# lym01803/FinalProject-LosslessImageCompression

Hardware: AMD Instinct MI355X
Metric: encode+decode Mpixels/s (imagenet64, bit-exact round trip) (higher is better)
Workload: dtype f32

## Files before the change

### finalproject-losslessimagecompression_amd/csrc/conv3_dx3.hip

```cpp
#include <hip/hip_runtime.h>
#include <stdint.h>
#include <stdlib.h>
#include <string.h>

#include <type_traits>
#include <utility>

#include "idf_cdf.h"
#include "idf_codec_internal.h"
#include "wino_common.h"

#pragma clang fp contract(off)

namespace idf {

typedef float d4 __attribute__((ext_vector_type(4)));
typedef _Float16 e4 __attribute__((ext_vector_type(4)));
typedef _Float16 e8 __attribute__((ext_vector_type(8)));
typedef unsigned int v4u __attribute__((ext_vector_type(4)));
typedef __bf16 b8 __attribute__((ext_vector_type(8)));

struct Dx3Args {
  const uint16_t* xs;
  int64_t P;
// ... 1062 lines not shown
                                                       const float* __restrict__ x, int64_t ld_x,
                                                       uint16_t* __restrict__ xb,
                                                       uint32_t* __restrict__ zero, int32_t nzero) {
  const int nq = ((c1 + 15) / 16 * 16 - c0) / 4;
  const int64_t g = (int64_t)blockIdx.x * blockDim.x + threadIdx.x;
  if (g < nzero) zero[g] = 0u;
  if (g >= P * nq) return;
  const int64_t pix = g / nq;
  const int c = c0 + 4 * (int)(g - pix * nq);
  d4 v = d4{0.f, 0.f, 0.f, 0.f};
  if (c < c1) v = *(const d4*)(x + pix * ld_x + c);
  typedef __bf16 b4 __attribute__((ext_vector_type(4)));
  *(b4*)((char*)xb + ((int64_t)(c >> 4) * P + pix) * 32 + (c & 15) * 2) = __builtin_convertvector(v, b4);
}

struct Dx3Plan {
  int ok, pitch, plane_kib, nbx, nby, ch, seg, segw, nseg, gut, wp, hp, nf, ngroup, split, tilew,
      xskip;
};

static int dx3_gcd(int a, int b) { return b ? dx3_gcd(b, a % b) : a; }

static Dx3Plan dx3_plan(int H, int W, int N, bool bf = false) {
  Dx3Plan p = {};
  p.tilew = 16;
  if (H < 1 || W < 1 || N < 1 || N > 1024) return p;
  const int nft = (N + 15) / 16;
  p.nf = nft <= 4 ? nft : 4;
  p.ngroup = (nft + p.nf - 1) / p.nf;
  if (W % 16 == 0) {
// ... 165 lines not shown
}

extern "C" int idf_dx3_head_init(void* stream, int64_t P, int32_t C0, const float* x, int64_t ld_x,
                                 const float* w, int32_t ldw, const float* bias, int32_t n_head,
                                 float* acc) {
  if (P <= 0) return P < 0 ? IDF_ERR_ARG : IDF_OK;
  if (!x || !w || !bias || !acc || n_head < 1 || n_head > 16 || C0 < 0 || C0 > 64 || (C0 & 3) ||
      (ld_x & 3) || (uintptr_t)x % 16 || (uintptr_t)acc % 16 || ldw < C0 || (ldw & 3) ||
      (uintptr_t)w % 16)
    return IDF_ERR_ARG;
  hipLaunchKernelGGL(dx3_head_init_kernel, dim3((unsigned)((P + 255) / 256)), dim3(256), 0,
                     (hipStream_t)stream, P, C0, x, ld_x, w, ldw, bias, n_head, acc);
  return idf_last_error();
}
#endif

static bool dxb_plan_ok(const Dx3Plan& p) {
  return p.ok && p.nf <= 3 && p.ngroup == 1 && (p.pitch == 18 || p.pitch == 10);
}

extern "C" int idf_conv3x3_dxb_supported(int32_t H, int32_t W, int32_t N) {
  return dxb_plan_ok(dx3_plan(H, W, N, true)) ? 1 : 0;
}

static bool dx3_plan_generic() {
  const char* e = getenv("IDF_DX3_PLAN");
  return e && !strcmp(e, "generic");
}

static int dx3_args(Dx3Args& g, Dx3Launch& sh, bool ml, bool bf, int32_t B, int32_t H, int32_t W,
// ... 283 lines not shown
```

### finalproject-losslessimagecompression_amd/csrc/flow_kernels.hip

```cpp
#include <hip/hip_runtime.h>
#include <stdint.h>

#include <algorithm>
#include <vector>

#include "idf_cdf.h"
#include "idf_codec_internal.h"

#pragma clang fp contract(off)

namespace idf {

typedef float floatx4 __attribute__((ext_vector_type(4)));

enum { MODE_DENSE = 0, MODE_CONV3 = 1 };
enum { EPI_STORE = 0, EPI_ACT = 1, EPI_COUPLE_ADD = 2, EPI_COUPLE_SUB = 3, EPI_PRIOR = 4,
       EPI_ACT_FOLD = 5 };

struct GemmArgs {
  int64_t P;
  int32_t K;
  int32_t N;
  const float* A;
  int64_t lda;
// ... 554 lines not shown
    t->used++;
  }
}

enum { COPY_NONE = 0, COPY_BF16_SHADOW, COPY_DX3_SPLIT, COPY_DXB };

struct BlockPlan {
  int8_t kind[IDF_MAX_DEPTH];
  bool wx3_first[IDF_MAX_DEPTH];
  bool fused;
  int head, head_init;
  int copy;
  int n_dx3;
  int dx3_nft;
  int conv_launches, setup_launches, head_launches;
  int64_t ld16, sh16;
  int nslab_xs;
  int64_t xs_bytes, off, need, hoff, bytes;
};

static int dense_block_plan(const IdfDenseBlock* blk, int32_t B, int32_t H, int32_t W, bool head,
                            BlockPlan* pl) {
  *pl = {};
  const int64_t P = (int64_t)B * H * W;
  const int depth = blk->depth;
  const bool dxb = blk->bf16 && blk->fold && blk->dxb && depth > 0 &&
                   idf_conv3x3_dxb_supported(H, W, blk->g_pad);
  bool dx3 = blk->fold && blk->wx3 && blk->dx3 && !blk->bf16 &&
             idf_conv3x3_dx3_supported(H, W, blk->g_pad);
  int n_dx3 = 0;
  while (dx3 && n_dx3 < depth && blk->dx3_w[n_dx3]) ++n_dx3;
  for (int i = n_dx3; dx3 && i < depth; ++i)
    if (blk->dx3_w[i]) return IDF_ERR_ARG;
  dx3 = dx3 && n_dx3 > 0;
// ... 37 lines not shown
  const bool wino = blk->fold && blk->wino && idf_conv3x3_wino_supported(H, W);
  for (int i = 0; i < depth; ++i) {
    int k = IDF_KIND_FOLD_GEMM;
    if (!blk->fold) k = IDF_KIND_UNFOLD;
    else if (dxb) k = IDF_KIND_DXB;
    else if (blk->bf16) k = IDF_KIND_BF16;
    else if (dx3 && i < n_dx3) k = IDF_KIND_DX3;
    else if (wino && blk->wino_u[i]) k = blk->wx3 && blk->wx3_u[i] ? IDF_KIND_WX3 : IDF_KIND_WINO;
    else if (blk->halo) k = IDF_KIND_HALO;
    pl->kind[i] = (int8_t)k;
    pl->wx3_first[i] = k == IDF_KIND_WX3 && (i == 0 || (dx3 && i == n_dx3));
  }
  pl->conv_launches = pl->fused ? 1 : blk->fold ? depth : 2 * depth;
  pl->setup_launches = (pl->copy != COPY_NONE) + (pl->head_init == IDF_HEAD_INIT_OWN_LAUNCH);
  pl->head_launches = pl->head == IDF_PLAN_HEAD_GEMM;
  return IDF_OK;
}

static bool block_args_ok(const IdfDenseBlock* blk, int32_t B, int32_t H, int32_t W) {
  return blk && blk->depth >= 0 && blk->depth <= IDF_MAX_DEPTH && B >= 0 && H >= 1 && W >= 1;
}

extern "C" int64_t idf_dense_block_dx3_tmp_bytes(const IdfDenseBlock* blk, int32_t B, int32_t H,
                                                  int32_t W) {
  BlockPlan pl;
  return block_args_ok(blk, B, H, W) && !dense_block_plan(blk, B, H, W, true, &pl) ? pl.bytes : -1;
}

extern "C" int idf_dense_block_plan(const IdfDenseBlock* blk, int32_t B, int32_t H, int32_t W,
                                    int32_t with_head, int32_t out[IDF_BLOCK_PLAN_N]) {
// ... 2 lines not shown
  if (!block_args_ok(blk, B, H, W)) return IDF_ERR_ARG;
  BlockPlan pl;
  if (int rc = dense_block_plan(blk, B, H, W, with_head != 0, &pl)) return rc;
  out[IDF_BLOCK_PLAN_FUSED] = pl.fused;
  out[IDF_BLOCK_PLAN_HEAD] = pl.head;
  out[IDF_BLOCK_PLAN_HEAD_INIT] = pl.head_init;
  out[IDF_BLOCK_PLAN_N_DX3] = pl.n_dx3;
  out[IDF_BLOCK_PLAN_CONV_LAUNCHES] = pl.conv_launches;
  out[IDF_BLOCK_PLAN_SETUP_LAUNCHES] = pl.setup_launches;
  out[IDF_BLOCK_PLAN_HEAD_LAUNCHES] = pl.head_launches;
  for (int i = 0; i < blk->depth; ++i) {
    out[IDF_BLOCK_PLAN_KIND0 + i] = pl.kind[i];
    if (pl.wx3_first[i]) out[IDF_BLOCK_PLAN_WX3_FIRST] |= (int32_t)(1u << i);
  }
  return IDF_OK;
}

static int dense_block_run_fused(void* stream, const IdfDenseBlock* blk, const BlockPlan& pl,
                                 int32_t B, int32_t H, int32_t W, float* feat, int64_t ld_feat,
                                 uint16_t* xs, const IdfDx3Head* hd, IdfTimer* timer) {
  const bool dxb = pl.copy == COPY_DXB;
  const int64_t P = (int64_t)B * H * W;
  int32_t C[16];
  const uint16_t* w[16];
  float ys[16];
  const float *b3[16], *vt[16], *bfu[16];
  double fl = 0.0;
  for (int i = 0; i < blk->depth; ++i) {
    C[i] = blk->k_in[i];
    w[i] = dxb ? blk->dxb_w[i] : blk->dx3_w[i];
// ... 29 lines not shown
  BlockPlan pl;
  if (int rc = dense_block_plan(blk, B, H, W, head != nullptr, &pl)) return rc;
  const int64_t tmp_floats = P * ld_tmp;
  const bool direct = pl.copy == COPY_DX3_SPLIT || pl.copy == COPY_DXB;
  if (pl.sh16 > tmp_floats || pl.bytes > tmp_floats * 4 || (direct && (uintptr_t)tmp % 256))
    return IDF_ERR_WORKSPACE;
  uint16_t* const xs = (uint16_t*)tmp;
  float* const ws = tmp + pl.sh16;
  char* const dws = (char*)tmp + pl.off;
  float* const hacc = pl.head == IDF_PLAN_HEAD_FUSED ? (float*)((char*)tmp + pl.hoff) : nullptr;
  const int c0 = blk->k_in[0];
  uint32_t* const ctr = pl.need > 0 ? (uint32_t*)dws : nullptr;
  const int32_t nctr =
      pl.need > 0 ? (int32_t)(idf_conv3x3_dx3_counter_bytes(B, H, W, blk->g_pad) / 4) : 0;
  int rc = IDF_OK;
  switch (pl.copy) {
    case COPY_BF16_SHADOW:
      rc = idf_f32_to_bf16_cols(stream, P, c0, (c0 + 7) / 8 * 8, feat, ld_feat, xs, pl.ld16);
      break;
    case COPY_DXB:
      rc = idf_dxb_cols(stream, P, 0, c0, feat, ld_feat, xs, pl.nslab_xs, ctr, nctr);
      break;
    case COPY_DX3_SPLIT:
      rc = pl.head_init == IDF_HEAD_INIT_IN_SPLIT
               ? idf_dx3_split_cols_head(stream, P, c0, feat, ld_feat, xs, pl.nslab_xs,
                                         blk->range_flag, ctr, nctr, blk->wh, blk->ldwh, blk->bh,
                                         blk->n_head, hacc)
               : idf_dx3_split_cols(stream, P, 0, c0, feat, ld_feat, xs, pl.nslab_xs,
                                    blk->range_flag, ctr, nctr);
      break;
  }
// ... 263 lines not shown
```

### finalproject-losslessimagecompression_amd/csrc/idf_codec_internal.h

```cpp
#pragma once
#include <hip/hip_runtime.h>
#include <stdint.h>

#include "../../include/idf_codec.h"

struct IdfDx3BlockDesc {
  int32_t bf;
  int32_t B, H, W, nlayers, N, nft, ldv, act, nslab_xs;
  float slope;
  uint16_t* xs;
  const int32_t* C;
  const uint16_t* const* w;
  const float* yscale;
  const float* const* b3;
  const float* const* vtap;
  const float* const* bfull;
  float* feat;
  int64_t ld_feat;
  uint32_t* flag;
  const IdfDx3Head* head;
  const float* hx;
  int64_t hld_x;
  int32_t hc0;
  const float* hb;
};
int idf_dx3_block_launch(void* stream, const IdfDx3BlockDesc* d);

#define IDF_FREQ_SCALE_ZERO ((int32_t)0x80000000)

static inline int idf_last_error() {
  hipError_t e = hipGetLastError();
  return e == hipSuccess ? IDF_OK : IDF_ERR_HIP;
}

namespace idf {

__device__ __forceinline__ int xcd_contiguous(int bid, int nwg) {
#ifdef IDF_XCD_OFF
  return bid;
#endif
  const int q = nwg / 8, r = nwg % 8;
// ... 38 lines not shown
```

### finalproject-losslessimagecompression_amd/idfcodec/_lib.py

```python
from __future__ import annotations

import ctypes
import os

import torch

HERE = os.path.dirname(os.path.abspath(__file__))
PKG = os.path.dirname(HERE)
REPO = os.path.dirname(PKG)
LIB_PATH = os.environ.get("IDF_LIB_PATH") or os.path.join(HERE, "libidfcodec.so")
HEADER = os.path.join(REPO, "include", "idf_codec.h")

IDF_OK = 0
IDF_ERR_UNSUPPORTED = 4
ERR_NAMES = {1: "IDF_ERR_ARG", 2: "IDF_ERR_HIP", 3: "IDF_ERR_WORKSPACE", 4: "IDF_ERR_UNSUPPORTED"}

STREAM_SCALE_ZERO = 1
STREAM_FREQ_ZERO = 2
STREAM_NEG_CDF = 4
STREAM_UNDERFLOW = 8
STREAM_OUT_OF_WINDOW = 16
STREAM_WORDS_LEFT = 32

ACT = {"ReLU": 0, "LeakyReLU": 1, "Tanh": 2, "None": 3}
# ... 10 lines not shown

class IdfDenseBlock(ctypes.Structure):
    _fields_ = [
        ("depth", i32), ("act", i32), ("slope", f32), ("g_pad", i32), ("g_alloc", i32),
        ("k_in", i32 * (MAX_DEPTH + 1)), ("n1_alloc", i32 * MAX_DEPTH), ("ldw1", i32 * MAX_DEPTH),
        ("ldw3", i32 * MAX_DEPTH), ("w1", P * MAX_DEPTH), ("b1", P * MAX_DEPTH),
        ("w3", P * MAX_DEPTH), ("b3", P * MAX_DEPTH), ("n_head", i32), ("nh_alloc", i32),
        ("ldwh", i32), ("wh", P), ("bh", P),
        ("c_real", i32 * (MAX_DEPTH + 1)), ("g_real", i32 * MAX_DEPTH),
        ("fold", i32), ("ldv", i32), ("vtap", P * MAX_DEPTH), ("bfull", P * MAX_DEPTH),
        ("halo", i32), ("wino", i32), ("wino_nft", i32), ("wino_u", P * MAX_DEPTH),
        ("bf16", i32), ("wb16", P * MAX_DEPTH),
        ("wx3", i32), ("wx3_yscale", f32 * MAX_DEPTH), ("wx3_u", P * MAX_DEPTH), ("range_flag", P),
        ("dx3", i32), ("dx3_yscale", f32 * MAX_DEPTH), ("dx3_w", P * MAX_DEPTH),
        ("fuse_head", i32), ("keep_feat", i32),
        ("dxb", i32), ("dxb_w", P * MAX_DEPTH), ("fuse_layers", i32),
    ]


class IdfHeadOut(ctypes.Structure):
    _fields_ = [
        ("mode", i32), ("out", P), ("ld_out", i64), ("base", P), ("ld_base", i64),
        ("n_mean", i32), ("mean", P), ("logscale", P), ("scale", P),
    ]


class IdfDx3Head(ctypes.Structure):
    _fields_ = [
        ("w", P), ("ldw", i32), ("n_head", i32), ("acc", P), ("last", i32), ("skip_f32", i32),
        ("out", IdfHeadOut),
    ]
# ... 13 lines not shown
                                                    P]),
    "idf_gather_words": (ctypes.c_int, [P, i64, P, P, P, P, P]),
    "idf_rans_host_workspace_bytes": (i64, [i64, i64]),
    "idf_rans_encode_on": (ctypes.c_int, [P, P, i64, P, i64, P, P, P, P, P, P]),
    "idf_rans_decode_on": (ctypes.c_int, [P, P, i64, P, P, i64, i64, P, P, P, P]),
    "idf_rans_encode": (ctypes.c_int, [P, i64, P, P, P, P, P, P]),
    "idf_rans_decode": (ctypes.c_int, [P, P, i64, i64, P, P, P, P]),
    "idf_log_prob": (ctypes.c_int, [P, i64, i64, P, P, P, i32, f32, P, P]),
    "idf_expf_glibc": (ctypes.c_int, [P, i64, P, P]),
    "idf_expf_checksum": (ctypes.c_int, [P, u64, u64, P]),
    "idf_rans_cdf_selfcheck": (ctypes.c_int, [P, u64, u64, P]),
    "idf_rans_part1_selfcheck": (ctypes.c_int, [P, u64, u64, P]),
    "idf_dense_block_f32": (ctypes.c_int, [P, P, i32, i32, i32, P, i64, P, i64, P]),
    "idf_dense_block_dx3_tmp_bytes": (i64, [P, i32, i32, i32]),
    "idf_dense_block_plan": (ctypes.c_int, [P, i32, i32, i32, i32, P]),
    "idf_dx3_block_supported": (ctypes.c_int, [i32, i32, i32, i32]),
    "idf_dx3_launch_info": (ctypes.c_int, [i32, i32, i32, i32, i32, i32, P]),
    "idf_gemm_launch_info": (ctypes.c_int, [i64, i32, P]),
    "idf_timer_create": (P, [i32]),
    "idf_timer_destroy": (None, [P]),
    "idf_timer_reset": (None, [P]),
    "idf_timer_summary": (ctypes.c_int, [P, i32, P, P, P]),
    "idf_dense_block_f32_timed": (ctypes.c_int, [P, P, i32, i32, i32, P, i64, P, i64, P, P]),
    "idf_conv1x1_f32": (ctypes.c_int, [P, i64, i32, i32, P, i64, P, i32, i32, P, P, i64, i32, i32,
                                       i32, P]),
    "idf_conv3x3_f32": (ctypes.c_int, [P, i32, i32, i32, i32, P, i64, P, i32, i32, P, i32, P, i64,
                                       i32, f32]),
    "idf_conv3x3_fold_f32": (ctypes.c_int, [P, i32, i32, i32, i32, P, i64, P, i32, i32, P, P, i32,
                                            P, i32, P, i64, i32, f32]),
    "idf_conv3x3_halo_workspace": (i64, [i32, i32, i32, i32, i32]),
# ... 147 lines not shown


def block_plan(desc: IdfDenseBlock, B: int, H: int, W: int, head: bool = True) -> dict:
    out = (ctypes.c_int32 * (len(BLOCK_PLAN_FIELDS) + MAX_DEPTH))()
    check(lib().idf_dense_block_plan(ctypes.byref(desc), B, H, W, int(head), out),
          "idf_dense_block_plan")
    p = dict(zip(BLOCK_PLAN_FIELDS, out))
    p["fused"] = bool(p["fused"])
    p["head"] = BLOCK_HEADS[p["head"]]
    p["head_init"] = BLOCK_HEAD_INITS[p["head_init"]]
    p["wx3_first"] = tuple(bool(p["wx3_first"] >> i & 1) for i in range(desc.depth))
    p["kind"] = tuple(BLOCK_KINDS[k] for k in out[len(BLOCK_PLAN_FIELDS):][:desc.depth])
    return p


GEMM_INFO_FIELDS = ("BN", "BM", "m_tiles", "n_tiles", "n_alloc_min")


def gemm_launch_info(P: int, N: int) -> dict:
    out = (ctypes.c_int32 * len(GEMM_INFO_FIELDS))()
    check(lib().idf_gemm_launch_info(P, N, out), "idf_gemm_launch_info")
    return dict(zip(GEMM_INFO_FIELDS, out))


def require_device(t: torch.Tensor, what: str = "tensor"):
    if not isinstance(t, torch.Tensor) or t.device.type != "cuda":
        raise IdfError(f"idfcodec: {what} must be a HIP device tensor (no CPU fallback)")


def new_stream(device=None, priority: int | None = None) -> torch.cuda.ExternalStream:
# ... 22 lines not shown
```

### finalproject-losslessimagecompression_amd/idfcodec/engine.py

```python
from __future__ import annotations

import collections
import ctypes
import os
from dataclasses import dataclass

import numpy as np
import torch

from . import _lib
from ._lib import IdfDenseBlock, IdfError, IdfHeadOut, check, lib, ptr
from .packing import PackedBlock, pack_dense_block_cached, round_up

FLOAT = 4
CONV_MODES = ("dx3", "dx3w16", "x3", "f32")
SPLIT_F16 = ("dx3", "dx3w16", "x3")
FOLD = os.environ.get("IDF_FOLD", "1") != "0"
HALO = os.environ.get("IDF_HALO", "1") != "0"
WINO = os.environ.get("IDF_WINO", "1") != "0"
WX3 = os.environ.get("IDF_WX3", "1") != "0"
DX3 = os.environ.get("IDF_DX3", "1") != "0"
_FL = os.environ.get("IDF_FUSE_LAYERS", "1")
FUSE_LAYERS = _FL != "0"
FUSE_LEVELS = None if _FL in ("0", "1") else {int(v) for v in _FL.split(",") if v}
# ... 71 lines not shown
            d.vtap[i] = self.vtap[i].data_ptr()
            d.bfull[i] = self.bfull[i].data_ptr()
        self.desc = d
        self.timer = None
        self.set_mode("dxb" if (self.dxb_w and DXB) else "bf16" if d.bf16 else
                      "dx3" if self.dx3_w else "x3")

    def set_mode(self, mode: str, dx3_level: bool = True, fuse_layers: bool = FUSE_LAYERS):
        d = self.desc
        d.wx3 = 1 if (mode in SPLIT_F16 and d.wino and self.wx3_u) else 0
        d.dx3 = 1 if (mode in ("dx3", "dx3w16") and dx3_level and d.wx3 and self.dx3_w) else 0
        d.dxb = 1 if (mode == "dxb" and d.bf16 and self.dxb_w) else 0
        d.fuse_head = 1 if ((mode == "dx3" and d.dx3) or d.dxb) else 0
        d.fuse_layers = 1 if fuse_layers else 0

    def run(self, stream, B, H, W, feat, ld_feat, tmp, ld_tmp, head: IdfHeadOut | None):
        h = ctypes.byref(head) if head else None
        if self.timer is not None:
            check(lib().idf_dense_block_f32_timed(stream, ctypes.byref(self.desc), B, H, W, feat,
                                                  ld_feat, tmp, ld_tmp, h, self.timer),
                  "idf_dense_block_f32_timed")
        else:
            check(lib().idf_dense_block_f32(stream, ctypes.byref(self.desc), B, H, W, feat, ld_feat,
                                            tmp, ld_tmp, h), "idf_dense_block_f32")


def head_couple(mode, out_ptr, ld):
    h = IdfHeadOut()
    h.mode = mode
    h.out = out_ptr
    h.ld_out = ld
    h.base = out_ptr
# ... 24 lines not shown
    prior_x_zero: bool

    @property
    def n_sym(self) -> int:
        return self.z * self.h * self.w


class FlowEngine:

    def __init__(self, model, device=None, fold: bool | None = None):
        self.device = torch.device(device or "cuda")
        self.precision = getattr(model, "idf_precision", "f32")
        if self.precision not in ("f32", "bf16"):
            raise ValueError(f"idf_precision must be 'f32' or 'bf16', not {self.precision!r}")
        self.fold = FOLD if fold is None else bool(fold)
        if self.precision == "bf16":
            self.fold = True
        self.wino = self.fold and WINO and self.precision == "f32" and any(
            lib().idf_conv3x3_wino_supported(model.H // s, model.W // s)
            for s in [model.blocks[0]["extend"].scale ** (l + 1) for l in range(model.nsplit)])
        self.wx3 = self.wino and WX3
        self.dx3 = self.wx3 and DX3 and any(
            lib().idf_conv3x3_dx3_supported(model.H // s, model.W // s, 48)
            for s in [model.blocks[0]["extend"].scale ** (l + 1) for l in range(model.nsplit)])
        self.range_flag = torch.zeros(1, dtype=torch.int32, device=self.device)
        sd = {k: v for k, v in model.state_dict().items()}
        self.conditional = type(model).__name__ == "ConditionalFlows"
        self.conv_for_cond = bool(getattr(model, "conv_for_cond", False))
        self.nflows = model.nflows
        self.nsplit = model.nsplit
# ... 71 lines not shown
        self._top_prior = {}
        self._set_mode_flags(self.conv_mode)

    def _dx3_level(self, l: int) -> bool:
        Lv = self.levels[l]
        return bool(lib().idf_conv3x3_dx3_supported(Lv.h, Lv.w, 48))

    def _dx3_cmax(self, l: int):
        return None

    def _dx3_level_in(self, l: int, mode: str) -> bool:
        return mode in ("dx3", "dx3w16") and self._dx3_level(l) and (
            mode == "dx3" or self.levels[l].w % 16 == 0)

    def block_plan(self, l: int, blk, B: int = 1, head: bool = True) -> dict:
        return _lib.block_plan(blk.desc, B, self.levels[l].h, self.levels[l].w, head)

    def dx3_layers(self, l: int, geom) -> int:
        blk = next(b for b in self.couple[l] + [self.prior[l]] if b.geom == geom)
        return self.block_plan(l, blk)["kind"].count("DX3")

    def fused_block(self, l: int, blk) -> bool:
        return self.block_plan(l, blk)["fused"]

    def _set_mode_flags(self, mode: str):
        for l, L in enumerate(self.levels):
            fuse = FUSE_LAYERS and (FUSE_LEVELS is None or L.h in FUSE_LEVELS)
            for b in self.couple[l] + [self.prior[l]]:
                b.set_mode(mode, self._dx3_level_in(l, mode), fuse)

    def set_conv_mode(self, mode: str):
        if self.precision == "bf16":
            if mode not in BF16_MODES or (mode == "dxb" and not self.dxb):
                raise ValueError(f"this bf16 engine runs conv modes "
                                 f"{BF16_MODES if self.dxb else ('bf16',)}, not {mode!r}")
        elif mode not in CONV_MODES:
            raise ValueError(f"conv mode must be one of {CONV_MODES}, not {mode!r}")
        elif mode == "x3" and not self.wx3:
            raise ValueError("this engine has no split-f16 (wx3) weights")
        elif mode in ("dx3", "dx3w16") and not self.dx3:
# ... 176 lines not shown
        s = _lib.stream_ptr(self.device)
        offs = self.sym_offsets(B)
        if self.conditional:
            self._prep_cond(ws, B, cond, s)
        if img is not None and img.numel() < B * self.H * self.W * 4:
            raise ValueError("img holds fewer than B pixel-major images")
        src, ld_src, H, W, C = ptr(ws["img"] if img is None else img), 4, self.H, self.W, self.C
        for l, Lv in enumerate(self.levels):
            ws["cur"][l] = 0
            P = B * Lv.h * Lv.w
            check(L.idf_squeeze(s, B, H, W, C, self.scale, src, ld_src, ptr(self._x(ws, l)), Lv.ldx),
                  "squeeze")
            for k in range(self.nflows):
                blk = self.couple[l][k]
                x, x2 = self._x(ws, l), self._x(ws, l, 1)
                check(L.idf_permute_couple_in(s, P, Lv.C, ptr(self.ids[l][k]), ptr(x), Lv.ldx, ptr(x2),
                                              Lv.ldx, Lv.a, blk.geom.a_pad, ptr(ws["feat"]),
                                              self.ld_feat), "permute")
                self._swap(ws, l)
                xo = ptr(x2) + Lv.a * FLOAT
                blk.run(s, B, Lv.h, Lv.w, ptr(ws["feat"]), self.ld_feat, ptr(ws["tmp"]),
                        self.tmp_pitch(ws, P), head_couple(_lib.EPI_COUPLE_ADD, xo, Lv.ldx))
                yield l
            x, x2 = self._x(ws, l), self._x(ws, l, 1)
            check(L.idf_permute_couple_in(s, P, Lv.C, ptr(self.ids[l][self.nflows]), ptr(x), Lv.ldx,
                                          ptr(x2), Lv.ldx, 0, 0, None, 0), "permute")
            self._swap(ws, l)
            x = self._x(ws, l)
            o = offs[l]
            check(L.idf_pm_to_nchw(s, B, Lv.z, Lv.h, Lv.w, ptr(x), Lv.ldx,
                                   ptr(ws["lat"]) + o * FLOAT), "pm_to_nchw")
            mean, logs, scale = (ptr(ws[k]) + o * FLOAT for k in ("mean", "logscale", "scale"))
            if Lv.prior_x_zero and not self.conditional:
                self._top_prior_cached(ws, B, s, o)
            else:
                self._prior(ws, B, l, s, mean, logs, scale, ptr(x) + Lv.z * FLOAT, Lv.ldx)
            if on_level is not None:
# ... 42 lines not shown
            P = B * Lv.h * Lv.w
            x = self._x(ws, l)
            o = offs[l]
            if pre_prior is not None:
                pre_prior(l)
            if priors:
                mean, logs, scale = (ptr(ws[k]) + o * FLOAT for k in ("mean", "logscale", "scale"))
                if Lv.prior_x_zero and not self.conditional:
                    self._top_prior_cached(ws, B, s, o)
                else:
                    self._prior(ws, B, l, s, mean, logs, scale, ptr(x) + Lv.z * FLOAT, Lv.ldx)
            decode_level(l, ws)
            yield l
            check(L.idf_nchw_to_pm(s, B, Lv.z, Lv.h, Lv.w, ptr(ws["lat"]) + o * FLOAT, ptr(x),
                                   Lv.ldx), "nchw_to_pm")
            x2 = self._x(ws, l, 1)
            check(L.idf_permute_couple_in(s, P, Lv.C, ptr(self.inv_ids[l][self.nflows]), ptr(x),
                                          Lv.ldx, ptr(x2), Lv.ldx, 0, 0, None, 0), "permute")
            self._swap(ws, l)
            for k in reversed(range(self.nflows)):
                blk = self.couple[l][k]
                x, x2 = self._x(ws, l), self._x(ws, l, 1)
                check(L.idf_copy_cols(s, P, Lv.a, blk.geom.a_pad, ptr(x), Lv.ldx, ptr(ws["feat"]),
                                      self.ld_feat), "copy cols")
                xo = ptr(x) + Lv.a * FLOAT
                blk.run(s, B, Lv.h, Lv.w, ptr(ws["feat"]), self.ld_feat, ptr(ws["tmp"]),
                        self.tmp_pitch(ws, P), head_couple(_lib.EPI_COUPLE_SUB, xo, Lv.ldx))
                check(L.idf_permute_couple_in(s, P, Lv.C, ptr(self.inv_ids[l][k]), ptr(x), Lv.ldx,
                                              ptr(x2), Lv.ldx, 0, 0, None, 0), "permute")
                self._swap(ws, l)
                yield l
            x = self._x(ws, l)
            if l > 0:
                Lp = self.levels[l - 1]
                dst, ldd = ptr(self._x(ws, l - 1)) + Lp.z * FLOAT, Lp.ldx
                Hh, Ww, Cc = Lp.h, Lp.w, Lp.rest
            else:
                dst, ldd, Hh, Ww, Cc = (ptr(ws["img"] if img is None else img), 4, self.H,
                                        self.W, self.C)
            check(L.idf_unsqueeze(s, B, Hh, Ww, Cc, self.scale, ptr(x), Lv.ldx, dst, ldd),
                  "unsqueeze")
        return ws

    def image_nchw(self, ws, B, out=None):
        if out is None:
            out = torch.empty((B, self.C, self.H, self.W), dtype=torch.float32, device=self.device)
# ... 18 lines not shown
```

### include/idf_codec.h

```cpp
#ifndef IDF_CODEC_H
#define IDF_CODEC_H

#include <stdint.h>

#ifdef __cplusplus
extern "C" {
#endif

#define IDF_OK 0
#define IDF_ERR_ARG 1
#define IDF_ERR_HIP 2
#define IDF_ERR_WORKSPACE 3
#define IDF_ERR_UNSUPPORTED 4

#define IDF_STREAM_SCALE_ZERO 1
#define IDF_STREAM_FREQ_ZERO 2
#define IDF_STREAM_NEG_CDF 4
#define IDF_STREAM_UNDERFLOW 8
#define IDF_STREAM_OUT_OF_WINDOW 16
#define IDF_STREAM_WORDS_LEFT 32

const char *idf_version(void);
int idf_device_count(void);

// ... 92 lines not shown
  const float *wino_u[IDF_MAX_DEPTH];
  int32_t bf16;
  const uint16_t *wb16[IDF_MAX_DEPTH];
  int32_t wx3;
  float wx3_yscale[IDF_MAX_DEPTH];
  const uint16_t *wx3_u[IDF_MAX_DEPTH];
  uint32_t *range_flag;
  int32_t dx3;
  float dx3_yscale[IDF_MAX_DEPTH];
  const uint16_t *dx3_w[IDF_MAX_DEPTH];
  int32_t fuse_head;
  int32_t keep_feat;
  int32_t dxb;
  const uint16_t *dxb_w[IDF_MAX_DEPTH];
  int32_t fuse_layers;
} IdfDenseBlock;

typedef struct IdfHeadOut {
  int32_t mode;
  float *out;
  int64_t ld_out;
  const float *base;
  int64_t ld_base;
  int32_t n_mean;
  float *mean;
  float *logscale;
  float *scale;
} IdfHeadOut;

int idf_dense_block_f32(void *stream, const IdfDenseBlock *blk, int32_t B, int32_t H, int32_t W,
// ... 15 lines not shown
  IDF_KIND_UNFOLD = 0, IDF_KIND_FOLD_GEMM, IDF_KIND_HALO, IDF_KIND_WINO, IDF_KIND_WX3,
  IDF_KIND_DX3, IDF_KIND_BF16, IDF_KIND_DXB
};
enum { IDF_PLAN_HEAD_NONE = 0, IDF_PLAN_HEAD_GEMM, IDF_PLAN_HEAD_FUSED };
enum {
  IDF_HEAD_INIT_NONE = 0, IDF_HEAD_INIT_IN_SPLIT, IDF_HEAD_INIT_OWN_LAUNCH, IDF_HEAD_INIT_IN_BLOCK
};
enum {
  IDF_BLOCK_PLAN_FUSED = 0, IDF_BLOCK_PLAN_HEAD, IDF_BLOCK_PLAN_HEAD_INIT, IDF_BLOCK_PLAN_N_DX3,
  IDF_BLOCK_PLAN_CONV_LAUNCHES, IDF_BLOCK_PLAN_SETUP_LAUNCHES, IDF_BLOCK_PLAN_HEAD_LAUNCHES,
  IDF_BLOCK_PLAN_WX3_FIRST, IDF_BLOCK_PLAN_KIND0,
  IDF_BLOCK_PLAN_N = IDF_BLOCK_PLAN_KIND0 + IDF_MAX_DEPTH
};
int idf_dense_block_plan(const IdfDenseBlock *blk, int32_t B, int32_t H, int32_t W,
                         int32_t with_head, int32_t out[IDF_BLOCK_PLAN_N]);

#define IDF_TAG_CONV1X1 0
#define IDF_TAG_CONV3X3 1
#define IDF_TAG_HEAD 2
typedef struct IdfTimer IdfTimer;
IdfTimer *idf_timer_create(int32_t capacity);
void idf_timer_destroy(IdfTimer *t);
void idf_timer_reset(IdfTimer *t);
int idf_timer_summary(IdfTimer *t, int32_t tag, double *total_ms, int64_t *count, double *flops);
int idf_dense_block_f32_timed(void *stream, const IdfDenseBlock *blk, int32_t B, int32_t H,
                              int32_t W, float *d_feat, int64_t ld_feat, float *d_tmp,
                              int64_t ld_tmp, const IdfHeadOut *head, IdfTimer *timer);

enum {
  IDF_GEMM_INFO_BN = 0, IDF_GEMM_INFO_BM, IDF_GEMM_INFO_M_TILES, IDF_GEMM_INFO_N_TILES,
// ... 293 lines not shown
```

Baseline: 21.73.

## Fuse coupling permute, feature copy, staging and head init into one glue kernel

Adds a couple_glue kernel that performs the channel permutation, writes the conditioning features, converts them into the split f16 hi/lo (or bf16) staging slabs for the dx3/dxb conv, zeroes the counters, and computes the head-init accumulator, all in one pass. Dense blocks get a 'prepared' flag so they skip their own setup copy launch, and the encode/decode loops in Python are restructured so the glue replaces the separate permute and copy_cols launches. This is meant to cut kernel launches and repeated global-memory passes per coupling layer. The cost is more complex plan bookkeeping and a heavier per-thread kernel, including a small serial head-init dot product.

New measurement: 21.85, median of 6. No clear change (+0.6%).

```diff
diff --git a/finalproject-losslessimagecompression_amd/csrc/conv3_dx3.hip b/finalproject-losslessimagecompression_amd/csrc/conv3_dx3.hip
--- a/finalproject-losslessimagecompression_amd/csrc/conv3_dx3.hip
+++ b/finalproject-losslessimagecompression_amd/csrc/conv3_dx3.hip
@@ -1100,6 +1100,67 @@
   *(b4*)((char*)xb + ((int64_t)(c >> 4) * P + pix) * 32 + (c & 15) * 2) = __builtin_convertvector(v, b4);
 }
 
+__global__ void __launch_bounds__(256) couple_glue_kernel(IdfCoupleGlue g, int vdst) {
+  const int nqx = (g.C + 3) / 4, nqs = (g.c1 + 15) / 16 * 4;
+  const int nq = nqx > nqs ? nqx : nqs;
+  const int64_t t = (int64_t)blockIdx.x * blockDim.x + threadIdx.x;
+  if (t < g.nzero) g.zero[t] = 0u;
+  if (t >= g.P * nq) return;
+  const int64_t pix = t / nq;
+  const int kq = (int)(t - pix * nq);
+  const int c = 4 * kq;
+  const float* sr = g.src + pix * g.ld_src;
+  if (g.acc && kq < 4) {
+    d4 h;
+#pragma unroll
+    for (int i = 0; i < 4; ++i) h[i] = 4 * kq + i < g.n_head ? g.hb[4 * kq + i] : 0.0f;
+    for (int cc = 0; cc < g.c1; cc += 4) {
+      d4 xv;
+#pragma unroll
+      for (int k = 0; k < 4; ++k) xv[k] = cc + k < g.a ? sr[g.ids[cc + k]] : 0.0f;
+#pragma unroll
+      for (int i = 0; i < 4; ++i) {
+        if (4 * kq + i >= g.n_head) break;
+        const d4 wv = *(const d4*)(g.hw + (int64_t)(4 * kq + i) * g.ldhw + cc);
+#pragma unroll
+        for (int k = 0; k < 4; ++k) h[i] = __builtin_fmaf(wv[k], xv[k], h[i]);
+      }
+    }
+    *(d4*)(g.acc + pix * 16 + 4 * kq) = h;
+  }
+  d4 e = d4{0.f, 0.f, 0.f, 0.f};
+#pragma unroll
+  for (int i = 0; i < 4; ++i)
+    if (c + i < g.C) e[i] = sr[g.ids[c + i]];
+  float* dr = g.dst + pix * g.ld_dst + c;
+  if (vdst && c + 4 <= g.C) {
+    *(d4*)dr = e;
+  } else {
+#pragma unroll
+    for (int i = 0; i < 4; ++i)
+      if (c + i < g.C) dr[i] = e[i];
+  }
+  if (kq >= nqs) return;
+  d4 v;
+#pragma unroll
+  for (int i = 0; i < 4; ++i) v[i] = c + i < g.a ? e[i] : 0.0f;
+  if (g.feat && c < g.c1) *(d4*)(g.feat + pix * g.ld_feat + c) = v;
+  if (g.bf) {
+    typedef __bf16 b4 __attribute__((ext_vector_type(4)));
+    *(b4*)((char*)g.xs + ((int64_t)(c >> 4) * g.P + pix) * 32 + (c & 15) * 2) =
+        __builtin_convertvector(v, b4);
+    return;
+  }
+  const e4 h = __builtin_convertvector(v, e4);
+  const e4 l = __builtin_convertvector(v - __builtin_convertvector(h, d4), e4);
+  char* p = (char*)g.xs + ((int64_t)(c >> 4) * 2 * g.P + pix) * 32 + (c & 15) * 2;
+  *(e4*)p = h;
+  *(e4*)(p + g.P * 32) = l;
+  const bool ok = fabsf(v[0]) < kDxInGuard && fabsf(v[1]) < kDxInGuard &&
+                  fabsf(v[2]) < kDxInGuard && fabsf(v[3]) < kDxInGuard;
+  if (!ok && g.flag) atomicOr(g.flag, 1u);
+}
+
 struct Dx3Plan {
   int ok, pitch, plane_kib, nbx, nby, ch, seg, segw, nseg, gut, wp, hp, nf, ngroup, split, tilew,
       xskip;
@@ -1295,6 +1356,31 @@
   return idf_last_error();
 }
 #endif
+
+int idf_couple_glue_launch(void* stream, const IdfCoupleGlue* gp) {
+  if (!gp) return IDF_ERR_ARG;
+  const IdfCoupleGlue& g = *gp;
+  if (g.P < 0 || g.nzero < 0 || (g.nzero && !g.zero)) return IDF_ERR_ARG;
+  if (g.C < 1 || g.a < 1 || g.a > g.c1 || g.a > g.C || (g.c1 & 3)) return IDF_ERR_ARG;
+  if (!g.ids || !g.src || !g.dst || g.ld_src < g.C || g.ld_dst < g.C) return IDF_ERR_ARG;
+  if (!g.xs || (g.c1 + 15) / 16 > g.nslab_xs) return IDF_ERR_ARG;
+  if (g.feat && (g.ld_feat < g.c1 || (g.ld_feat & 3) || (uintptr_t)g.feat % 16)) return IDF_ERR_ARG;
+  if (g.acc && (g.bf || !g.hw || !g.hb || g.n_head < 1 || g.n_head > 16 || g.c1 > 64 ||
+                g.ldhw < g.c1 || (g.ldhw & 3) || (uintptr_t)g.hw % 16 || (uintptr_t)g.acc % 16))
+    return IDF_ERR_ARG;
+  if (g.P == 0) {
+    if (g.nzero) return hipMemsetAsync(g.zero, 0, 4 * (size_t)g.nzero, (hipStream_t)stream) == hipSuccess
+                            ? IDF_OK : IDF_ERR_HIP;
+    return IDF_OK;
+  }
+  const int nqx = (g.C + 3) / 4, nqs = (g.c1 + 15) / 16 * 4;
+  int64_t n = g.P * (nqx > nqs ? nqx : nqs);
+  if (n < g.nzero) n = g.nzero;
+  const int vdst = !(g.ld_dst & 3) && !((uintptr_t)g.dst % 16);
+  hipLaunchKernelGGL(couple_glue_kernel, dim3((unsigned)((n + 255) / 256)), dim3(256), 0,
+                     (hipStream_t)stream, g, vdst);
+  return idf_last_error();
+}
 
 static bool dxb_plan_ok(const Dx3Plan& p) {
   return p.ok && p.nf <= 3 && p.ngroup == 1 && (p.pitch == 18 || p.pitch == 10);
diff --git a/finalproject-losslessimagecompression_amd/csrc/flow_kernels.hip b/finalproject-losslessimagecompression_amd/csrc/flow_kernels.hip
--- a/finalproject-losslessimagecompression_amd/csrc/flow_kernels.hip
+++ b/finalproject-losslessimagecompression_amd/csrc/flow_kernels.hip
@@ -592,10 +592,14 @@
   int n_dx3;
   int dx3_nft;
   int conv_launches, setup_launches, head_launches;
+  bool can_prepare;
+  bool feat_in;
   int64_t ld16, sh16;
   int nslab_xs;
   int64_t xs_bytes, off, need, hoff, bytes;
 };
+
+static bool k0_ok(const IdfDenseBlock* blk) { return blk->k_in[0] > 0 && !(blk->k_in[0] & 3); }
 
 static int dense_block_plan(const IdfDenseBlock* blk, int32_t B, int32_t H, int32_t W, bool head,
                             BlockPlan* pl) {
@@ -663,6 +667,12 @@
   pl->conv_launches = pl->fused ? 1 : blk->fold ? depth : 2 * depth;
   pl->setup_launches = (pl->copy != COPY_NONE) + (pl->head_init == IDF_HEAD_INIT_OWN_LAUNCH);
   pl->head_launches = pl->head == IDF_PLAN_HEAD_GEMM;
+  pl->can_prepare = (dx3 || dxb) && k0_ok(blk) && pl->head_init != IDF_HEAD_INIT_OWN_LAUNCH;
+  pl->feat_in = !(pl->head_init == IDF_HEAD_INIT_IN_SPLIT && !blk->keep_feat);
+  if (blk->prepared) {
+    if (!pl->can_prepare || !head) return IDF_ERR_ARG;
+    pl->setup_launches = 0;
+  }
   return IDF_OK;
 }
 
@@ -695,6 +705,55 @@
     if (pl.wx3_first[i]) out[IDF_BLOCK_PLAN_WX3_FIRST] |= (int32_t)(1u << i);
   }
   return IDF_OK;
+}
+
+static int32_t plan_nctr(const BlockPlan& pl, const IdfDenseBlock* blk, int32_t B, int32_t H,
+                         int32_t W) {
+  return pl.need > 0 ? (int32_t)(idf_conv3x3_dx3_counter_bytes(B, H, W, blk->g_pad) / 4) : 0;
+}
+
+extern "C" int idf_dense_block_tmp_layout(const IdfDenseBlock* blk, int32_t B, int32_t H, int32_t W,
+                                          int32_t with_head, int64_t out[IDF_TMP_LAYOUT_N]) {
+  if (!out) return IDF_ERR_ARG;
+  for (int i = 0; i < IDF_TMP_LAYOUT_N; ++i) out[i] = 0;
+  if (!block_args_ok(blk, B, H, W)) return IDF_ERR_ARG;
+  BlockPlan pl;
+  if (int rc = dense_block_plan(blk, B, H, W, with_head != 0, &pl)) return rc;
+  out[IDF_TMP_LAYOUT_XS_BYTES] = pl.xs_bytes;
+  out[IDF_TMP_LAYOUT_NSLAB] = pl.nslab_xs;
+  out[IDF_TMP_LAYOUT_WS_OFF] = pl.off;
+  out[IDF_TMP_LAYOUT_WS_BYTES] = pl.need;
+  out[IDF_TMP_LAYOUT_NCTR] = plan_nctr(pl, blk, B, H, W);
+  out[IDF_TMP_LAYOUT_HEAD_OFF] = pl.hoff;
+  out[IDF_TMP_LAYOUT_BYTES] = pl.bytes;
+  out[IDF_TMP_LAYOUT_FEAT_IN] = pl.feat_in;
+  out[IDF_TMP_LAYOUT_CAN_PREPARE] = pl.can_prepare;
+  return IDF_OK;
+}
+
+extern "C" int idf_couple_glue(void* stream, const IdfDenseBlock* blk, int32_t B, int32_t H,
+                               int32_t W, int32_t C, const int32_t* ids, const float* src,
+                               int64_t ld_src, float* dst, int64_t ld_dst, int32_t a, float* feat,
+                               int64_t ld_feat, float* tmp, int64_t ld_tmp) {
+  if (!block_args_ok(blk, B, H, W) || !tmp || ld_tmp < 0) return IDF_ERR_ARG;
+  BlockPlan pl;
+  if (int rc = dense_block_plan(blk, B, H, W, true, &pl)) return rc;
+  if (!pl.can_prepare || (pl.feat_in && !feat)) return IDF_ERR_ARG;
+  const int64_t P = (int64_t)B * H * W;
+  if (pl.bytes > P * ld_tmp * 4 || (uintptr_t)tmp % 256) return IDF_ERR_WORKSPACE;
+  IdfCoupleGlue g = {};
+  g.P = P; g.C = C; g.a = a; g.c1 = blk->k_in[0]; g.bf = pl.copy == COPY_DXB;
+  g.nslab_xs = pl.nslab_xs; g.nzero = plan_nctr(pl, blk, B, H, W);
+  g.ids = ids; g.src = src; g.ld_src = ld_src; g.dst = dst; g.ld_dst = ld_dst;
+  g.xs = (uint16_t*)tmp;
+  g.flag = g.bf ? nullptr : blk->range_flag;
+  g.zero = g.nzero ? (uint32_t*)((char*)tmp + pl.off) : nullptr;
+  g.feat = pl.feat_in ? feat : nullptr; g.ld_feat = ld_feat;
+  if (pl.head_init == IDF_HEAD_INIT_IN_SPLIT) {
+    g.hw = blk->wh; g.ldhw = blk->ldwh; g.n_head = blk->n_head; g.hb = blk->bh;
+    g.acc = (float*)((char*)tmp + pl.hoff);
+  }
+  return idf_couple_glue_launch(stream, &g);
 }
 
 static int dense_block_run_fused(void* stream, const IdfDenseBlock* blk, const BlockPlan& pl,
@@ -754,7 +813,7 @@
   const int32_t nctr =
       pl.need > 0 ? (int32_t)(idf_conv3x3_dx3_counter_bytes(B, H, W, blk->g_pad) / 4) : 0;
   int rc = IDF_OK;
-  switch (pl.copy) {
+  switch (blk->prepared ? COPY_NONE : pl.copy) {
     case COPY_BF16_SHADOW:
       rc = idf_f32_to_bf16_cols(stream, P, c0, (c0 + 7) / 8 * 8, feat, ld_feat, xs, pl.ld16);
       break;
diff --git a/finalproject-losslessimagecompression_amd/csrc/idf_codec_internal.h b/finalproject-losslessimagecompression_amd/csrc/idf_codec_internal.h
--- a/finalproject-losslessimagecompression_amd/csrc/idf_codec_internal.h
+++ b/finalproject-losslessimagecompression_amd/csrc/idf_codec_internal.h
@@ -25,6 +25,26 @@
   const float* hb;
 };
 int idf_dx3_block_launch(void* stream, const IdfDx3BlockDesc* d);
+
+struct IdfCoupleGlue {
+  int64_t P;
+  int32_t C, a, c1, bf, nslab_xs, nzero;
+  const int32_t* ids;
+  const float* src;
+  int64_t ld_src;
+  float* dst;
+  int64_t ld_dst;
+  uint16_t* xs;
+  uint32_t* flag;
+  uint32_t* zero;
+  float* feat;
+  int64_t ld_feat;
+  const float* hw;
+  int32_t ldhw, n_head;
+  const float* hb;
+  float* acc;
+};
+int idf_couple_glue_launch(void* stream, const IdfCoupleGlue* g);
 
 #define IDF_FREQ_SCALE_ZERO ((int32_t)0x80000000)
 
diff --git a/finalproject-losslessimagecompression_amd/idfcodec/_lib.py b/finalproject-losslessimagecompression_amd/idfcodec/_lib.py
--- a/finalproject-losslessimagecompression_amd/idfcodec/_lib.py
+++ b/finalproject-losslessimagecompression_amd/idfcodec/_lib.py
@@ -48,7 +48,7 @@
         ("wx3", i32), ("wx3_yscale", f32 * MAX_DEPTH), ("wx3_u", P * MAX_DEPTH), ("range_flag", P),
         ("dx3", i32), ("dx3_yscale", f32 * MAX_DEPTH), ("dx3_w", P * MAX_DEPTH),
         ("fuse_head", i32), ("keep_feat", i32),
-        ("dxb", i32), ("dxb_w", P * MAX_DEPTH), ("fuse_layers", i32),
+        ("dxb", i32), ("dxb_w", P * MAX_DEPTH), ("fuse_layers", i32), ("prepared", i32),
     ]
 
 
@@ -92,6 +92,9 @@
     "idf_dense_block_f32": (ctypes.c_int, [P, P, i32, i32, i32, P, i64, P, i64, P]),
     "idf_dense_block_dx3_tmp_bytes": (i64, [P, i32, i32, i32]),
     "idf_dense_block_plan": (ctypes.c_int, [P, i32, i32, i32, i32, P]),
+    "idf_dense_block_tmp_layout": (ctypes.c_int, [P, i32, i32, i32, i32, P]),
+    "idf_couple_glue": (ctypes.c_int, [P, P, i32, i32, i32, i32, P, P, i64, P, i64, i32, P, i64, P,
+                                       i64]),
     "idf_dx3_block_supported": (ctypes.c_int, [i32, i32, i32, i32]),
     "idf_dx3_launch_info": (ctypes.c_int, [i32, i32, i32, i32, i32, i32, P]),
     "idf_gemm_launch_info": (ctypes.c_int, [i64, i32, P]),
@@ -269,6 +272,19 @@
     return p
 
 
+TMP_LAYOUT_FIELDS = ("xs_bytes", "nslab", "ws_off", "ws_bytes", "nctr", "head_off", "bytes",
+                     "feat_in", "can_prepare")
+
+
+def tmp_layout(desc: IdfDenseBlock, B: int, H: int, W: int, head: bool = True) -> dict:
+    out = (ctypes.c_int64 * len(TMP_LAYOUT_FIELDS))()
+    check(lib().idf_dense_block_tmp_layout(ctypes.byref(desc), B, H, W, int(head), out),
+          "idf_dense_block_tmp_layout")
+    p = dict(zip(TMP_LAYOUT_FIELDS, out))
+    p["feat_in"], p["can_prepare"] = bool(p["feat_in"]), bool(p["can_prepare"])
+    return p
+
+
 GEMM_INFO_FIELDS = ("BN", "BM", "m_tiles", "n_tiles", "n_alloc_min")
 
 
diff --git a/finalproject-losslessimagecompression_amd/idfcodec/engine.py b/finalproject-losslessimagecompression_amd/idfcodec/engine.py
--- a/finalproject-losslessimagecompression_amd/idfcodec/engine.py
+++ b/finalproject-losslessimagecompression_amd/idfcodec/engine.py
@@ -109,8 +109,10 @@
         d.fuse_head = 1 if ((mode == "dx3" and d.dx3) or d.dxb) else 0
         d.fuse_layers = 1 if fuse_layers else 0
 
-    def run(self, stream, B, H, W, feat, ld_feat, tmp, ld_tmp, head: IdfHeadOut | None):
+    def run(self, stream, B, H, W, feat, ld_feat, tmp, ld_tmp, head: IdfHeadOut | None,
+            prepared: bool = False):
         h = ctypes.byref(head) if head else None
+        self.desc.prepared = 1 if prepared else 0
         if self.timer is not None:
             check(lib().idf_dense_block_f32_timed(stream, ctypes.byref(self.desc), B, H, W, feat,
                                                   ld_feat, tmp, ld_tmp, h, self.timer),
@@ -165,6 +167,8 @@
         if self.precision not in ("f32", "bf16"):
             raise ValueError(f"idf_precision must be 'f32' or 'bf16', not {self.precision!r}")
         self.fold = FOLD if fold is None else bool(fold)
+        self.glue = os.environ.get("IDF_GLUE", "1") != "0"
+        self._glue_ok = {}
         if self.precision == "bf16":
             self.fold = True
         self.wino = self.fold and WINO and self.precision == "f32" and any(
@@ -266,7 +270,33 @@
             mode == "dx3" or self.levels[l].w % 16 == 0)
 
     def block_plan(self, l: int, blk, B: int = 1, head: bool = True) -> dict:
-        return _lib.block_plan(blk.desc, B, self.levels[l].h, self.levels[l].w, head)
+        blk.desc.prepared = 1 if head and self._glue_block(l, blk) else 0
+        try:
+            return _lib.block_plan(blk.desc, B, self.levels[l].h, self.levels[l].w, head)
+        finally:
+            blk.desc.prepared = 0
+
+    def _glue_block(self, l: int, blk) -> bool:
+        if not self.glue or blk not in self.couple[l]:
+            return False
+        key = (l, self.couple[l].index(blk))
+        hit = self._glue_ok.get(key)
+        if hit is None:
+            Lv = self.levels[l]
+            blk.desc.prepared = 0
+            try:
+                hit = _lib.tmp_layout(blk.desc, 1, Lv.h, Lv.w)["can_prepare"]
+            except IdfError:
+                hit = False
+            self._glue_ok[key] = hit
+        return hit
+
+    def _glue(self, ws, l, B, blk, ids, x, x2, s):
+        Lv = self.levels[l]
+        check(lib().idf_couple_glue(s, ctypes.byref(blk.desc), B, Lv.h, Lv.w, Lv.C, ptr(ids),
+                                    ptr(x), Lv.ldx, ptr(x2), Lv.ldx, Lv.a, ptr(ws["feat"]),
+                                    self.ld_feat, ptr(ws["tmp"]),
+                                    self.tmp_pitch(ws, B * Lv.h * Lv.w)), "couple glue")
 
     def dx3_layers(self, l: int, geom) -> int:
         blk = next(b for b in self.couple[l] + [self.prior[l]] if b.geom == geom)
@@ -276,6 +306,7 @@
         return self.block_plan(l, blk)["fused"]
 
     def _set_mode_flags(self, mode: str):
+        self._glue_ok.clear()
         for l, L in enumerate(self.levels):
             fuse = FUSE_LAYERS and (FUSE_LEVELS is None or L.h in FUSE_LEVELS)
             for b in self.couple[l] + [self.prior[l]]:
@@ -482,13 +513,17 @@
             for k in range(self.nflows):
                 blk = self.couple[l][k]
                 x, x2 = self._x(ws, l), self._x(ws, l, 1)
-                check(L.idf_permute_couple_in(s, P, Lv.C, ptr(self.ids[l][k]), ptr(x), Lv.ldx, ptr(x2),
-                                              Lv.ldx, Lv.a, blk.geom.a_pad, ptr(ws["feat"]),
-                                              self.ld_feat), "permute")
+                pre = self._glue_block(l, blk)
+                if pre:
+                    self._glue(ws, l, B, blk, self.ids[l][k], x, x2, s)
+                else:
+                    check(L.idf_permute_couple_in(s, P, Lv.C, ptr(self.ids[l][k]), ptr(x), Lv.ldx,
+                                                  ptr(x2), Lv.ldx, Lv.a, blk.geom.a_pad,
+                                                  ptr(ws["feat"]), self.ld_feat), "permute")
                 self._swap(ws, l)
                 xo = ptr(x2) + Lv.a * FLOAT
                 blk.run(s, B, Lv.h, Lv.w, ptr(ws["feat"]), self.ld_feat, ptr(ws["tmp"]),
-                        self.tmp_pitch(ws, P), head_couple(_lib.EPI_COUPLE_ADD, xo, Lv.ldx))
+                        self.tmp_pitch(ws, P), head_couple(_lib.EPI_COUPLE_ADD, xo, Lv.ldx), pre)
                 yield l
             x, x2 = self._x(ws, l), self._x(ws, l, 1)
             check(L.idf_permute_couple_in(s, P, Lv.C, ptr(self.ids[l][self.nflows]), ptr(x), Lv.ldx,
@@ -561,22 +596,27 @@
             yield l
             check(L.idf_nchw_to_pm(s, B, Lv.z, Lv.h, Lv.w, ptr(ws["lat"]) + o * FLOAT, ptr(x),
                                    Lv.ldx), "nchw_to_pm")
-            x2 = self._x(ws, l, 1)
-            check(L.idf_permute_couple_in(s, P, Lv.C, ptr(self.inv_ids[l][self.nflows]), ptr(x),
-                                          Lv.ldx, ptr(x2), Lv.ldx, 0, 0, None, 0), "permute")
-            self._swap(ws, l)
-            for k in reversed(range(self.nflows)):
-                blk = self.couple[l][k]
+            for k in reversed(range(-1, self.nflows)):
+                blk = self.couple[l][k] if k >= 0 else None
+                nxt = k >= 0 and self._glue_block(l, blk)
                 x, x2 = self._x(ws, l), self._x(ws, l, 1)
-                check(L.idf_copy_cols(s, P, Lv.a, blk.geom.a_pad, ptr(x), Lv.ldx, ptr(ws["feat"]),
-                                      self.ld_feat), "copy cols")
+                if nxt:
+                    self._glue(ws, l, B, blk, self.inv_ids[l][k + 1], x, x2, s)
+                else:
+                    check(L.idf_permute_couple_in(s, P, Lv.C, ptr(self.inv_ids[l][k + 1]), ptr(x),
+                                                  Lv.ldx, ptr(x2), Lv.ldx, 0, 0, None, 0), "permute")
+                self._swap(ws, l)
+                if k < self.nflows - 1:
+                    yield l
+                if k < 0:
+                    break
+                x = self._x(ws, l)
+                if not nxt:
+                    check(L.idf_copy_cols(s, P, Lv.a, blk.geom.a_pad, ptr(x), Lv.ldx,
+                                          ptr(ws["feat"]), self.ld_feat), "copy cols")
                 xo = ptr(x) + Lv.a * FLOAT
                 blk.run(s, B, Lv.h, Lv.w, ptr(ws["feat"]), self.ld_feat, ptr(ws["tmp"]),
-                        self.tmp_pitch(ws, P), head_couple(_lib.EPI_COUPLE_SUB, xo, Lv.ldx))
-                check(L.idf_permute_couple_in(s, P, Lv.C, ptr(self.inv_ids[l][k]), ptr(x), Lv.ldx,
-                                              ptr(x2), Lv.ldx, 0, 0, None, 0), "permute")
-                self._swap(ws, l)
-                yield l
+                        self.tmp_pitch(ws, P), head_couple(_lib.EPI_COUPLE_SUB, xo, Lv.ldx), nxt)
             x = self._x(ws, l)
             if l > 0:
                 Lp = self.levels[l - 1]
diff --git a/include/idf_codec.h b/include/idf_codec.h
--- a/include/idf_codec.h
+++ b/include/idf_codec.h
@@ -130,6 +130,7 @@
   int32_t dxb;
   const uint16_t *dxb_w[IDF_MAX_DEPTH];
   int32_t fuse_layers;
+  int32_t prepared;
 } IdfDenseBlock;
 
 typedef struct IdfHeadOut {
@@ -175,6 +176,18 @@
 };
 int idf_dense_block_plan(const IdfDenseBlock *blk, int32_t B, int32_t H, int32_t W,
                          int32_t with_head, int32_t out[IDF_BLOCK_PLAN_N]);
+enum {
+  IDF_TMP_LAYOUT_XS_BYTES = 0, IDF_TMP_LAYOUT_NSLAB, IDF_TMP_LAYOUT_WS_OFF, IDF_TMP_LAYOUT_WS_BYTES,
+  IDF_TMP_LAYOUT_NCTR, IDF_TMP_LAYOUT_HEAD_OFF, IDF_TMP_LAYOUT_BYTES, IDF_TMP_LAYOUT_FEAT_IN,
+  IDF_TMP_LAYOUT_CAN_PREPARE, IDF_TMP_LAYOUT_N
+};
+int idf_dense_block_tmp_layout(const IdfDenseBlock *blk, int32_t B, int32_t H, int32_t W,
+                               int32_t with_head, int64_t out[IDF_TMP_LAYOUT_N]);
+
+int idf_couple_glue(void *stream, const IdfDenseBlock *blk, int32_t B, int32_t H, int32_t W,
+                    int32_t C, const int32_t *d_ids, const float *d_src, int64_t ld_src,
+                    float *d_dst, int64_t ld_dst, int32_t a, float *d_feat, int64_t ld_feat,
+                    float *d_tmp, int64_t ld_tmp);
 
 #define IDF_TAG_CONV1X1 0
 #define IDF_TAG_CONV3X3 1
```
